# madmann91/bvh

Measured on AMD Instinct MI355X. Metric: Mrays/s closest-hit (1M-tri scene), higher is better.
Workload: dtype f32; 1 GPU; soup_1m: 1,000,000-triangle random soup (M3), worst-case incoherent; robust traversal, DefaultBuilder with thread pool (mini-trees) Quality::High built on the GPU (the reference's default configuration is thread pool + High); rays reordered for coherence inside the timed pass (library default for this tree size); tris=1000000, nodes=1866439, ray_batches=4, parallelism=single GPU, launched_by=single process

## Files before the change

### bvh_amd/csrc/trace_body.inc

```
#ifndef BVH_TRACE_COOP
#define BVH_TRACE_COOP false
#endif
    constexpr int kDepth = kLdsDepth;
    constexpr int kSpill = 64 - kDepth;
    __shared__ uint32_t lds_stack[kDepth * kBlock];
    uint32_t spill[kSpill];
    const int tid = threadIdx.x;
    const int lane = tid & (kWave - 1);
    const uint64_t lanes_below = (uint64_t{1} << lane) - 1;

    bool have = false, done = false, drained = false, nan_ray = false;
    uint32_t part = a.parts > 1 ? blockIdx.x % a.parts : 0, parts_left = a.parts;
    unsigned long long ray_id = 0;
    T org[3], dir[3], inv[3], aux[3];
    T tmin = 0, tmax = 0;
    uint32_t oct[3] = {0, 0, 0};
    uint32_t top = 0, sp = 0;
    uint32_t hit_prim = BVH_AMD_INVALID;
    T hit_t = 0, hit_u = 0, hit_v = 0;
    unsigned long long n_pairs = 0, n_tests = 0, n_leaves = 0;
#if defined(BVH_AMD_DEVELOPER) && defined(__HIPCC__)
    unsigned long long wt_begin = 0, wt_last_refill = 0, wt_rays = 0, wt_refill_ticks = 0, wt_refills = 0;
    if (a.wave_times) wt_begin = __builtin_amdgcn_s_memrealtime();
#endif

    auto deep_slot = [&](uint32_t i) { return a.deep + (size_t{blockIdx.x} * kBlock + tid) * a.deep_cap + i; };
    auto push = [&](uint32_t v) {
        if (sp < kDepth) lds_stack[sp * kBlock + tid] = v;
        else if (!Deep) spill[min(sp - kDepth, static_cast<uint32_t>(kSpill - 1))] = v;
        else if (sp < kDepth + kSpill) spill[sp - kDepth] = v;
        else *deep_slot(min(sp - (kDepth + kSpill), a.deep_cap - 1)) = v;
        ++sp;
    };
    auto pop = [&]() -> uint32_t {
        --sp;
        uint32_t v = lds_word(&lds_stack[min(sp, static_cast<uint32_t>(kDepth - 1)) * kBlock + tid]);
        if (sp >= kDepth) {
            if (!Deep) v = spill[min(sp - kDepth, static_cast<uint32_t>(kSpill - 1))];
            else if (sp < kDepth + kSpill) v = spill[sp - kDepth];
            else v = *deep_slot(min(sp - (kDepth + kSpill), a.deep_cap - 1));
        }
        return v;
    };

    for (;;) {
        const uint64_t idle = __ballot(!have);
        const int n_idle = __popcll(idle);
        if (!drained && (n_idle >= a.refill_threshold || n_idle == kWave)) {
#if defined(BVH_AMD_DEVELOPER) && defined(__HIPCC__)
            unsigned long long wt_t0 = 0;
            if (a.wave_times) wt_t0 = __builtin_amdgcn_s_memrealtime();
#endif
            unsigned long long base = 0, part_end = a.n;
            if (a.one_shot) {
                base = (static_cast<unsigned long long>(blockIdx.x) * (kBlock / kWave) + (tid >> 6)) * kWave;
                drained = true;
            } else {
                if (lane == 0) base = atomicAdd(a.work + part * kTicketStride, static_cast<unsigned long long>(n_idle));
                base = __shfl(base, 0) + part * a.part_size;
                part_end = min(a.n, (part + 1ull) * a.part_size);
                if (base + n_idle >= part_end) {
                    part = part + 1 == a.parts ? 0 : part + 1;
                    if (--parts_left == 0) drained = true;
                } else if (a.stagger && part_end - (base + n_idle) < static_cast<unsigned long long>(a.stagger) * ((blockIdx.x * 8u) / gridDim.x)) {
                    drained = true;
                }
            }
            if (!have) {
                const unsigned long long ticket = base + __popcll(idle & lanes_below);
                if (ticket < part_end) {
                    const bool once = (a.stream_hints & 1u) != 0;
                    const unsigned long long my = a.order ? (once ? load_word_nt(a.order + ticket) : a.order[ticket]) : ticket;
                    T r[8];
                    if (D == 3) { if (once) load_ray_nt(a.rays + 8 * my, r); else load_ray(a.rays + 8 * my, r); }
                    else {
                        T q[6];
                        load_ray2(a.rays + 6 * my, q);
                        r[0] = q[0]; r[1] = q[1]; r[2] = T(0); r[3] = q[2]; r[4] = q[3]; r[5] = T(0); r[6] = q[4]; r[7] = q[5];
                    }
#pragma unroll
                    for (int k = 0; k < D; ++k) {
                        org[k] = r[k]; dir[k] = r[3 + k];
                        T d = dir[k];
                        T iv = Robust ? T(1) / d
                                      : (Num<T>::abs_(d) <= Num<T>::kEps ? Num<T>::copysign_(Num<T>::kMax, d) : T(1) / d);
                        inv[k] = iv;
                        aux[k] = Robust ? (Num<T>::finite(iv) ? Num<T>::bump2(iv) : iv) : (-iv) * org[k];
                        oct[k] = Num<T>::sign(d) ? 1u : 0u;
                    }
                    tmin = r[6]; tmax = r[7];
                    nan_ray = !(tmin == tmin) || !(tmax == tmax);
                    ray_id = my;
                    have = true; done = false;
                    sp = 0;
                    top = a.root_index;
                    hit_prim = BVH_AMD_INVALID; hit_t = tmax; hit_u = 0; hit_v = 0;
                }
            }
#if defined(BVH_AMD_DEVELOPER) && defined(__HIPCC__)
            if (a.wave_times) {
                asm volatile("s_waitcnt vmcnt(0)" ::: "memory");
                wt_last_refill = __builtin_amdgcn_s_memrealtime(); wt_rays += __popcll(__ballot(have)) - (kWave - n_idle);
                wt_refill_ticks += wt_last_refill - wt_t0; ++wt_refills;
            }
#endif
        }
        if (__ballot(have) == 0) {
            if (drained) break;
            continue;
        }

        for (;;) {
            const bool inner = have && !done && (top & kCountMask) == 0;
            const uint64_t inner_mask = __ballot(inner);
            if (!inner_mask) break;
            const int parked = __popcll(__ballot(have && !done && (top & kCountMask) != 0));
            if (parked >= a.leaf_threshold) break;
            T lb[6], rb[6];
            uint32_t li = 0, ri = 0;
            if constexpr (BVH_TRACE_COOP) coop_load_pair(a.pairs, a.pair_bytes, inner ? (top >> (kCountBits + 1)) : 0xFFFFFFFFu, lane, lb, rb, li, ri);
            if (inner) {
                if constexpr (!BVH_TRACE_COOP) load_pair(a.pairs + (top >> (kCountBits + 1)), lb, rb, li, ri);
                if (Stats) ++n_pairs;
                T l0 = tmin, l1 = tmax, r0 = tmin, r1 = tmax;
#pragma unroll
                for (int k = 0; k < D; ++k) {
                    const T ln = oct[k] ? lb[2 * k + 1] : lb[2 * k], lf = oct[k] ? lb[2 * k] : lb[2 * k + 1];
                    const T rn = oct[k] ? rb[2 * k + 1] : rb[2 * k], rf = oct[k] ? rb[2 * k] : rb[2 * k + 1];
                    T la, lz, ra, rz;
                    if (Robust) {
                        la = (ln - org[k]) * inv[k]; lz = (lf - org[k]) * aux[k];
                        ra = (rn - org[k]) * inv[k]; rz = (rf - org[k]) * aux[k];
                    } else {
                        la = Num<T>::fma_(ln, inv[k], aux[k]); lz = Num<T>::fma_(lf, inv[k], aux[k]);
                        ra = Num<T>::fma_(rn, inv[k], aux[k]); rz = Num<T>::fma_(rf, inv[k], aux[k]);
                    }
                    l0 = Num<T>::max_num(la, l0); l1 = Num<T>::min_num(lz, l1);
                    r0 = Num<T>::max_num(ra, r0); r1 = Num<T>::min_num(rz, r1);
                }
                const bool hl = !nan_ray && l0 <= l1, hr = !nan_ray && r0 <= r1;
                if (hl) {
                    uint32_t near_i = li;
                    if (hr) {
                        uint32_t far_i = ri;
                        if (!Any && l0 > r0) { near_i = ri; far_i = li; }
                        push(far_i);
                    }
                    top = near_i;
                } else if (hr) {
                    top = ri;
                } else if (sp == 0) {
                    done = true;
                } else {
                    top = pop();
                }
            }
        }

        if (have && !done && (top & kCountMask) != 0) {
            const uint32_t first = top >> kCountBits, count = top & kCountMask;
            if (Stats) ++n_leaves;
            for (uint32_t i = first; i < first + count; ++i) {
                if (Stats) ++n_tests;
                if (Leaf == LEAF_TRIANGLE) {
                    T p[12];
                    load_prim12(a.prims + static_cast<unsigned long long>(a.prim_stride) * i, p);
                    const T c0 = p[0] - org[0], c1 = p[1] - org[1], c2 = p[2] - org[2];
                    const T rx = dir[1] * c2 - dir[2] * c1, ry = dir[2] * c0 - dir[0] * c2, rz = dir[0] * c1 - dir[1] * c0;
                    const T inv_det = T(1) / dot3(p[9], p[10], p[11], dir[0], dir[1], dir[2]);
                    const T u = dot3(rx, ry, rz, p[6], p[7], p[8]) * inv_det;
                    const T v = dot3(rx, ry, rz, p[3], p[4], p[5]) * inv_det;
                    const T w = T(1) - u - v;
                    const T tol = -Num<T>::kEps;
                    if (u >= tol && v >= tol && w >= tol) {
                        const T t = dot3(p[9], p[10], p[11], c0, c1, c2) * inv_det;
                        if (t >= tmin && t <= tmax) { tmax = t; hit_t = t; hit_u = u; hit_v = v; hit_prim = i; }
                    }
                } else {
                    T qa, qb, qc;
                    if (D == 3) {
                        T s[4];
                        load_prim4(a.prims + 4ull * i, s);
                        const T o0 = org[0] - s[0], o1 = org[1] - s[1], o2 = org[2] - s[2];
                        qa = dot3(dir[0], dir[1], dir[2], dir[0], dir[1], dir[2]);
                        qb = T(2) * dot3(dir[0], dir[1], dir[2], o0, o1, o2);
                        qc = dot3(o0, o1, o2, o0, o1, o2) - s[3] * s[3];
                    } else {
                        const T* s = a.prims + 3ull * i;
                        const T o0 = org[0] - s[0], o1 = org[1] - s[1];
                        qa = dot2(dir[0], dir[1], dir[0], dir[1]);
                        qb = T(2) * dot2(dir[0], dir[1], o0, o1);
                        qc = dot2(o0, o1, o0, o1) - s[2] * s[2];
                    }
                    const T delta = qb * qb - T(4) * qa * qc;
                    if (delta >= 0) {
                        const T iv = -T(0.5) / qa;
                        const T root = Num<T>::sqrt_(delta);
                        const T t0 = pick_max((qb + root) * iv, tmin);
                        const T t1 = pick_min((qb - root) * iv, tmax);
                        if (t0 <= t1) { tmax = t0; hit_t = t0; hit_u = t1; hit_v = 0; hit_prim = i; }
                    }
                }
            }
            if (Any && hit_prim != BVH_AMD_INVALID) done = true;
            else if (sp == 0) done = true;
            else top = pop();
        }

        if (have && done) {
            if (a.stream_hints & 1u) store_hit_nt(a.hits + ray_id, hit_prim, hit_t, hit_u, hit_v);
            else store_hit(a.hits + ray_id, hit_prim, hit_t, hit_u, hit_v);
            have = false;
        }
    }

#if defined(BVH_AMD_DEVELOPER) && defined(__HIPCC__)
    if (a.wave_times && lane == 0) {
        uint32_t xcc = 0;
        asm volatile("s_getreg_b32 %0, hwreg(HW_REG_XCC_ID)" : "=s"(xcc));
        unsigned long long* w = a.wave_times + 6ull * (blockIdx.x * (kBlock / kWave) + (tid >> 6));
        w[0] = wt_begin; w[1] = wt_last_refill; w[2] = __builtin_amdgcn_s_memrealtime(); w[3] = (static_cast<unsigned long long>(xcc & 0xFu) << 32) | (wt_rays & 0xFFFFFFFFull);
        w[4] = wt_refill_ticks; w[5] = wt_refills;
    }
#endif
    if (Stats) {
#pragma unroll
        for (int off = 32; off > 0; off >>= 1) {
            n_pairs += __shfl_down(n_pairs, off);
            n_tests += __shfl_down(n_tests, off);
            n_leaves += __shfl_down(n_leaves, off);
        }
        if (lane == 0) {
            atomicAdd(&a.counters->node_pairs, n_pairs);
            atomicAdd(&a.counters->prim_tests, n_tests);
            atomicAdd(&a.counters->leaves, n_leaves);
        }
    }
```

### bvh_amd/csrc/trace_device.h

```cpp
#pragma once

#if defined(__HIPCC__)
#define BVH_AMD_KEEP_APART(v) asm volatile("" : "+v"(v))
#else
#define BVH_AMD_KEEP_APART(v) asm volatile("" : "+r"(v))
#endif

namespace bvh_amd {

namespace {

constexpr int kBlock = 256;
constexpr int kLdsDepth = 20;
constexpr int kRefillThreshold = 36;
constexpr int kRefillThresholdSmall = 20;
constexpr int kLeafThreshold = 12;
constexpr int kCoopRefillAny = 20, kCoopLeafAny = 20;
constexpr int kCoopRefillHeavy = 12, kCoopLeafHeavy = 12;


template <typename T> struct Num;
template <> struct Num<float> {
    static constexpr float kMax = 3.402823466e+38f, kEps = 1.1920928955078125e-07f;
    __device__ static bool finite(float x) { return (__float_as_uint(x) & 0x7F800000u) != 0x7F800000u; }
    __device__ static float bump2(float x) { return __uint_as_float(__float_as_uint(x) + 2u); }
    __device__ static bool sign(float x) { return (__float_as_uint(x) >> 31) != 0; }
    __device__ static float fma_(float a, float b, float c) { return __builtin_fmaf(a, b, c); }
    __device__ static float sqrt_(float x) { return __builtin_sqrtf(x); }
    __device__ static float abs_(float x) { return __builtin_fabsf(x); }
    __device__ static float copysign_(float a, float b) { return __builtin_copysignf(a, b); }
    __device__ static float max_num(float a, float b) { return __builtin_fmaxf(a, b); }
    __device__ static float min_num(float a, float b) { return __builtin_fminf(a, b); }
};
template <> struct Num<double> {
    static constexpr double kMax = 1.7976931348623157e+308, kEps = 2.220446049250313e-16;
    __device__ static bool finite(double x) {
        return (static_cast<uint32_t>(__double_as_longlong(x) >> 32) & 0x7FF00000u) != 0x7FF00000u;
    }
    __device__ static double bump2(double x) { return __longlong_as_double(__double_as_longlong(x) + 2ll); }
    __device__ static bool sign(double x) { return (__double_as_longlong(x) >> 63) != 0; }
    __device__ static double fma_(double a, double b, double c) { return __builtin_fma(a, b, c); }
    __device__ static double sqrt_(double x) { return __builtin_sqrt(x); }
    __device__ static double abs_(double x) { return __builtin_fabs(x); }
    __device__ static double copysign_(double a, double b) { return __builtin_copysign(a, b); }
    __device__ static double max_num(double a, double b) { return __builtin_fmax(a, b); }
    __device__ static double min_num(double a, double b) { return __builtin_fmin(a, b); }
};

template <typename T> __device__ inline T pick_min(T a, T b) { return a < b ? a : b; }
template <typename T> __device__ inline T pick_max(T a, T b) { return a > b ? a : b; }

template <typename T> __device__ inline T dot3(T a0, T a1, T a2, T b0, T b1, T b2) {
    return ((T(0) + a0 * b0) + a1 * b1) + a2 * b2;
}
__device__ inline uint32_t lds_word(const uint32_t* shared) {
#if defined(__HIP_DEVICE_COMPILE__)
    typedef __attribute__((address_space(3))) const volatile uint32_t LdsWord;
    return *(LdsWord*)shared;
#else
    return *shared;
#endif
}

template <typename T> __device__ inline T dot2(T a0, T a1, T b0, T b1) { return (T(0) + a0 * b0) + a1 * b1; }

constexpr uint32_t kTicketStride = 16;

template <typename T>
struct TraceArgs {
    const PairNode<T>* pairs;
    const T* prims;
    const T* rays;
    typename HitOf<T>::Type* hits;
    unsigned long long n;
    unsigned long long* work;
    unsigned long long part_size;
    uint32_t parts;
    bvh_amd_counters* counters;
    const uint32_t* order;
    uint32_t* deep;
    uint32_t deep_cap;
    uint32_t root_index;
    int refill_threshold;
    int leaf_threshold;
    uint32_t coop;
    uint32_t prim_stride;
    uint32_t stream_hints;
    uint32_t stagger;
    uint32_t one_shot;
    unsigned long long* wave_times;
    uint32_t pair_bytes = 0;
};

__device__ inline void load_pair(const PairNode<float>* p, float (&lb)[6], float (&rb)[6], uint32_t& li, uint32_t& ri) {
    const float4* q = reinterpret_cast<const float4*>(p);
    float4 a = q[0], b = q[1], c = q[2];
    uint2 d = reinterpret_cast<const uint2*>(p)[6];
    lb[0] = a.x; lb[1] = a.y; lb[2] = a.z; lb[3] = a.w; lb[4] = b.x; lb[5] = b.y;
    rb[0] = b.z; rb[1] = b.w; rb[2] = c.x; rb[3] = c.y; rb[4] = c.z; rb[5] = c.w;
    li = d.x; ri = d.y;
}
__device__ inline void load_pair(const PairNode<double>* p, double (&lb)[6], double (&rb)[6], uint32_t& li, uint32_t& ri) {
    const double2* q = reinterpret_cast<const double2*>(p);
#pragma unroll
    for (int i = 0; i < 3; ++i) { double2 v = q[i]; lb[2 * i] = v.x; lb[2 * i + 1] = v.y; }
#pragma unroll
    for (int i = 0; i < 3; ++i) { double2 v = q[3 + i]; rb[2 * i] = v.x; rb[2 * i + 1] = v.y; }
    uint2 d = reinterpret_cast<const uint2*>(p)[12];
    li = d.x; ri = d.y;
}

#if defined(__HIPCC__)
template <int CTRL> __device__ inline uint32_t quad_perm(uint32_t v) {
    return static_cast<uint32_t>(__builtin_amdgcn_mov_dpp(static_cast<int>(v), CTRL, 0xF, 0xF, true));
}
template <bool ByTwo> __device__ inline void quad_exchange4(uint32_t (&a)[4], uint32_t (&b)[4]) {
    const uint64_t lower = ByTwo ? 0x3333333333333333ull : 0x5555555555555555ull;
    uint32_t n0, n1, n2, n3;
    if (ByTwo)
        asm("s_nop 1\n\ts_mov_b64 vcc, %12\n\t"
            "v_cndmask_b32_dpp %0, %4, %8, vcc quad_perm:[2,3,0,1] row_mask:0xf bank_mask:0xf\n\t"
            "v_cndmask_b32_dpp %1, %5, %9, vcc quad_perm:[2,3,0,1] row_mask:0xf bank_mask:0xf\n\t"
            "v_cndmask_b32_dpp %2, %6, %10, vcc quad_perm:[2,3,0,1] row_mask:0xf bank_mask:0xf\n\t"
            "v_cndmask_b32_dpp %3, %7, %11, vcc quad_perm:[2,3,0,1] row_mask:0xf bank_mask:0xf\n\t"
            "s_not_b64 vcc, vcc\n\t"
            "v_cndmask_b32_dpp %4, %8, %4, vcc quad_perm:[2,3,0,1] row_mask:0xf bank_mask:0xf\n\t"
            "v_cndmask_b32_dpp %5, %9, %5, vcc quad_perm:[2,3,0,1] row_mask:0xf bank_mask:0xf\n\t"
            "v_cndmask_b32_dpp %6, %10, %6, vcc quad_perm:[2,3,0,1] row_mask:0xf bank_mask:0xf\n\t"
            "v_cndmask_b32_dpp %7, %11, %7, vcc quad_perm:[2,3,0,1] row_mask:0xf bank_mask:0xf"
            : "=&v"(n0), "=&v"(n1), "=&v"(n2), "=&v"(n3), "+v"(b[0]), "+v"(b[1]), "+v"(b[2]), "+v"(b[3])
            : "v"(a[0]), "v"(a[1]), "v"(a[2]), "v"(a[3]), "s"(lower) : "vcc", "scc");
    else
        asm("s_nop 1\n\ts_mov_b64 vcc, %12\n\t"
            "v_cndmask_b32_dpp %0, %4, %8, vcc quad_perm:[1,0,3,2] row_mask:0xf bank_mask:0xf\n\t"
            "v_cndmask_b32_dpp %1, %5, %9, vcc quad_perm:[1,0,3,2] row_mask:0xf bank_mask:0xf\n\t"
            "v_cndmask_b32_dpp %2, %6, %10, vcc quad_perm:[1,0,3,2] row_mask:0xf bank_mask:0xf\n\t"
            "v_cndmask_b32_dpp %3, %7, %11, vcc quad_perm:[1,0,3,2] row_mask:0xf bank_mask:0xf\n\t"
            "s_not_b64 vcc, vcc\n\t"
            "v_cndmask_b32_dpp %4, %8, %4, vcc quad_perm:[1,0,3,2] row_mask:0xf bank_mask:0xf\n\t"
            "v_cndmask_b32_dpp %5, %9, %5, vcc quad_perm:[1,0,3,2] row_mask:0xf bank_mask:0xf\n\t"
            "v_cndmask_b32_dpp %6, %10, %6, vcc quad_perm:[1,0,3,2] row_mask:0xf bank_mask:0xf\n\t"
            "v_cndmask_b32_dpp %7, %11, %7, vcc quad_perm:[1,0,3,2] row_mask:0xf bank_mask:0xf"
            : "=&v"(n0), "=&v"(n1), "=&v"(n2), "=&v"(n3), "+v"(b[0]), "+v"(b[1]), "+v"(b[2]), "+v"(b[3])
            : "v"(a[0]), "v"(a[1]), "v"(a[2]), "v"(a[3]), "s"(lower) : "vcc", "scc");
    a[0] = n0; a[1] = n1; a[2] = n2; a[3] = n3;
}
#elif defined(BVH_HOST_WAVE64)
template <int CTRL> inline uint32_t quad_perm(uint32_t v) {
    const int l = static_cast<int>(threadIdx.x) & 63;
    return wave_read(v, (l & ~3) | ((CTRL >> (2 * (l & 3))) & 3), true);
}
template <bool ByTwo> inline void quad_exchange4(uint32_t (&a)[4], uint32_t (&b)[4]) {
    const int l = static_cast<int>(threadIdx.x) & 63, bit = ByTwo ? 2 : 1, partner = l ^ bit;
    const bool lower = (l & bit) == 0;
    for (int i = 0; i < 4; ++i) {
        const uint32_t pa = wave_read(a[i], partner, true), pb = wave_read(b[i], partner, true);
        const uint32_t na = lower ? a[i] : pb, nb = lower ? pa : b[i];
        a[i] = na; b[i] = nb;
    }
}
#endif
constexpr uint32_t kNoRecordAt = 0xFFFFFFFFu << 6;
#if defined(__HIPCC__)
using PairRsrc = __amdgpu_buffer_rsrc_t;
__device__ inline PairRsrc pair_rsrc(const void* base, uint32_t bytes) {
    return __builtin_amdgcn_make_buffer_rsrc(const_cast<void*>(base), 0, static_cast<int>(bytes), 0x00020000);
}
__device__ inline uint4 load_chunk(PairRsrc r, uint32_t at) {
    const auto v = __builtin_amdgcn_raw_buffer_load_b128(r, static_cast<int>(at), 0, 0);
    return uint4{v[0], v[1], v[2], v[3]};
}
#elif defined(BVH_HOST_WAVE64)
struct PairRsrc { const char* base; };
inline PairRsrc pair_rsrc(const void* base, uint32_t) { return PairRsrc{static_cast<const char*>(base)}; }
inline uint4 load_chunk(PairRsrc r, uint32_t at) {
    if (at >= kNoRecordAt) return uint4{0, 0, 0, 0};
    return *reinterpret_cast<const uint4*>(r.base + at);
}
#endif
#if defined(__HIPCC__) || defined(BVH_HOST_WAVE64)
__device__ inline void coop_load_pair(const PairNode<float>* pairs, uint32_t pair_bytes, uint32_t want, int lane, float (&lb)[6], float (&rb)[6], uint32_t& li, uint32_t& ri) {
    const uint32_t at = want << 6, chunk = (static_cast<uint32_t>(lane) & 3u) * 16u;
    const PairRsrc r = pair_rsrc(pairs, pair_bytes);
    const uint4 c0 = load_chunk(r, quad_perm<0x00>(at) | chunk), c1 = load_chunk(r, quad_perm<0x55>(at) | chunk);
    const uint4 c2 = load_chunk(r, quad_perm<0xAA>(at) | chunk), c3 = load_chunk(r, quad_perm<0xFF>(at) | chunk);
    uint32_t v0[4] = {c0.x, c0.y, c0.z, c0.w}, v1[4] = {c1.x, c1.y, c1.z, c1.w}, v2[4] = {c2.x, c2.y, c2.z, c2.w}, v3[4] = {c3.x, c3.y, c3.z, c3.w};
    quad_exchange4<false>(v0, v1); quad_exchange4<false>(v2, v3);
    quad_exchange4<true>(v0, v2); quad_exchange4<true>(v1, v3);
    lb[0] = __uint_as_float(v0[0]); lb[1] = __uint_as_float(v0[1]); lb[2] = __uint_as_float(v0[2]); lb[3] = __uint_as_float(v0[3]);
    lb[4] = __uint_as_float(v1[0]); lb[5] = __uint_as_float(v1[1]); rb[0] = __uint_as_float(v1[2]); rb[1] = __uint_as_float(v1[3]);
    rb[2] = __uint_as_float(v2[0]); rb[3] = __uint_as_float(v2[1]); rb[4] = __uint_as_float(v2[2]); rb[5] = __uint_as_float(v2[3]);
    li = v3[0]; ri = v3[1];
}
__device__ inline void coop_load_pair(const PairNode<double>* pairs, uint32_t, uint32_t want, int lane, double (&lb)[6], double (&rb)[6], uint32_t& li, uint32_t& ri) {
    constexpr uint32_t kNone = 0xFFFFFFFFu;
    const uint32_t j = static_cast<uint32_t>(lane) & 3u;
    const uint32_t o0 = quad_perm<0x00>(want), o1 = quad_perm<0x55>(want), o2 = quad_perm<0xAA>(want), o3 = quad_perm<0xFF>(want);
    const char* base = reinterpret_cast<const char*>(pairs);
    const uint32_t chunk = j * 16u;
    uint4 c0 = {0, 0, 0, 0}, c1 = {0, 0, 0, 0}, c2 = {0, 0, 0, 0}, c3 = {0, 0, 0, 0}, d0 = {0, 0, 0, 0}, d1 = {0, 0, 0, 0}, d2 = {0, 0, 0, 0}, d3 = {0, 0, 0, 0};
    if (o0 != kNone) { c0 = *reinterpret_cast<const uint4*>(base + (o0 * 128u + chunk)); d0 = *reinterpret_cast<const uint4*>(base + (o0 * 128u + 64u + chunk)); }
    if (o1 != kNone) { c1 = *reinterpret_cast<const uint4*>(base + (o1 * 128u + chunk)); d1 = *reinterpret_cast<const uint4*>(base + (o1 * 128u + 64u + chunk)); }
    if (o2 != kNone) { c2 = *reinterpret_cast<const uint4*>(base + (o2 * 128u + chunk)); d2 = *reinterpret_cast<const uint4*>(base + (o2 * 128u + 64u + chunk)); }
    if (o3 != kNone) { c3 = *reinterpret_cast<const uint4*>(base + (o3 * 128u + chunk)); d3 = *reinterpret_cast<const uint4*>(base + (o3 * 128u + 64u + chunk)); }
    uint32_t v0[4] = {c0.x, c0.y, c0.z, c0.w}, v1[4] = {c1.x, c1.y, c1.z, c1.w}, v2[4] = {c2.x, c2.y, c2.z, c2.w}, v3[4] = {c3.x, c3.y, c3.z, c3.w};
    uint32_t w0[4] = {d0.x, d0.y, d0.z, d0.w}, w1[4] = {d1.x, d1.y, d1.z, d1.w}, w2[4] = {d2.x, d2.y, d2.z, d2.w}, w3[4] = {d3.x, d3.y, d3.z, d3.w};
    quad_exchange4<false>(v0, v1); quad_exchange4<false>(v2, v3);
    quad_exchange4<true>(v0, v2); quad_exchange4<true>(v1, v3);
    quad_exchange4<false>(w0, w1); quad_exchange4<false>(w2, w3);
    quad_exchange4<true>(w0, w2); quad_exchange4<true>(w1, w3);
    auto dbl = [](uint32_t lo, uint32_t hi) { return __longlong_as_double(static_cast<long long>((static_cast<unsigned long long>(hi) << 32) | lo)); };
    lb[0] = dbl(v0[0], v0[1]); lb[1] = dbl(v0[2], v0[3]); lb[2] = dbl(v1[0], v1[1]); lb[3] = dbl(v1[2], v1[3]);
    lb[4] = dbl(v2[0], v2[1]); lb[5] = dbl(v2[2], v2[3]); rb[0] = dbl(v3[0], v3[1]); rb[1] = dbl(v3[2], v3[3]);
    rb[2] = dbl(w0[0], w0[1]); rb[3] = dbl(w0[2], w0[3]); rb[4] = dbl(w1[0], w1[1]); rb[5] = dbl(w1[2], w1[3]);
    li = w2[0]; ri = w2[1];
    (void)w3;
}
#else
template <typename T> inline void coop_load_pair(const PairNode<T>* p, uint32_t, uint32_t want, int, T (&lb)[6], T (&rb)[6], uint32_t& li, uint32_t& ri) {
    if (want != 0xFFFFFFFFu) load_pair(p + want, lb, rb, li, ri);
}
#endif

__device__ inline void load_prim12(const float* p, float (&v)[12]) {
    const float4* q = reinterpret_cast<const float4*>(p);
    float4 a = q[0], b = q[1], c = q[2];
    v[0] = a.x; v[1] = a.y; v[2] = a.z; v[3] = a.w; v[4] = b.x; v[5] = b.y; v[6] = b.z; v[7] = b.w;
    v[8] = c.x; v[9] = c.y; v[10] = c.z; v[11] = c.w;
}
__device__ inline void load_prim12(const double* p, double (&v)[12]) {
    const double2* q = reinterpret_cast<const double2*>(p);
#pragma unroll
    for (int i = 0; i < 6; ++i) { double2 t = q[i]; v[2 * i] = t.x; v[2 * i + 1] = t.y; }
}
__device__ inline void load_prim4(const float* p, float (&v)[4]) {
    float4 a = *reinterpret_cast<const float4*>(p);
    v[0] = a.x; v[1] = a.y; v[2] = a.z; v[3] = a.w;
}
__device__ inline void load_prim4(const double* p, double (&v)[4]) {
    const double2* q = reinterpret_cast<const double2*>(p);
    double2 a = q[0], b = q[1];
    v[0] = a.x; v[1] = a.y; v[2] = b.x; v[3] = b.y;
}
__device__ inline void load_ray(const float* p, float (&v)[8]) {
    const float4* q = reinterpret_cast<const float4*>(p);
    float4 a = q[0], b = q[1];
    v[0] = a.x; v[1] = a.y; v[2] = a.z; v[3] = a.w; v[4] = b.x; v[5] = b.y; v[6] = b.z; v[7] = b.w;
}
__device__ inline void load_ray(const double* p, double (&v)[8]) {
    const double2* q = reinterpret_cast<const double2*>(p);
#pragma unroll
    for (int i = 0; i < 4; ++i) { double2 t = q[i]; v[2 * i] = t.x; v[2 * i + 1] = t.y; }
}
__device__ inline void load_ray_nt(const float* p, float (&v)[8]) {
#if defined(__HIP_DEVICE_COMPILE__)
    typedef float f4 __attribute__((ext_vector_type(4)));
    const f4* q = reinterpret_cast<const f4*>(p);
    const f4 a = __builtin_nontemporal_load(q), b = __builtin_nontemporal_load(q + 1);
    v[0] = a.x; v[1] = a.y; v[2] = a.z; v[3] = a.w; v[4] = b.x; v[5] = b.y; v[6] = b.z; v[7] = b.w;
#else
    load_ray(p, v);
#endif
}
__device__ inline void load_ray_nt(const double* p, double (&v)[8]) { load_ray(p, v); }
__device__ inline uint32_t load_word_nt(const uint32_t* p) {
#if defined(__HIP_DEVICE_COMPILE__)
    return __builtin_nontemporal_load(p);
#else
    return *p;
#endif
}
__device__ inline void load_ray2(const float* p, float (&v)[6]) {
    const float2* q = reinterpret_cast<const float2*>(p);
    float2 a = q[0], b = q[1], c = q[2];
    v[0] = a.x; v[1] = a.y; v[2] = b.x; v[3] = b.y; v[4] = c.x; v[5] = c.y;
}
__device__ inline void load_ray2(const double* p, double (&v)[6]) {
    const double2* q = reinterpret_cast<const double2*>(p);
#pragma unroll
    for (int i = 0; i < 3; ++i) { double2 t = q[i]; v[2 * i] = t.x; v[2 * i + 1] = t.y; }
}
__device__ inline void store_hit(bvh_hit3f* out, uint32_t prim, float t, float u, float v) {
    *reinterpret_cast<float4*>(out) = make_float4(__uint_as_float(prim), t, u, v);
}
__device__ inline void store_hit(bvh_hit3d* out, uint32_t prim, double t, double u, double v) {
    double2* q = reinterpret_cast<double2*>(out);
    q[0] = make_double2(__longlong_as_double(static_cast<long long>(prim)), t);
    q[1] = make_double2(u, v);
}
__device__ inline void store_hit_nt(bvh_hit3f* out, uint32_t prim, float t, float u, float v) {
#if defined(__HIP_DEVICE_COMPILE__)
    typedef float f4 __attribute__((ext_vector_type(4)));
    f4 h; h.x = __uint_as_float(prim); h.y = t; h.z = u; h.w = v;
    __builtin_nontemporal_store(h, reinterpret_cast<f4*>(out));
#else
    store_hit(out, prim, t, u, v);
#endif
}
__device__ inline void store_hit_nt(bvh_hit3d* out, uint32_t prim, double t, double u, double v) { store_hit(out, prim, t, u, v); }

}

}
```

Baseline: 2438 Mrays/s.

## Rewrite inner-node traversal step with wave-mask logic and packed f32 slab math

Rewrites the inner BVH traversal loop so that control decisions (hit left/right, swap, push, pop, termination) are computed as wave-wide ballot masks. Stack pointer updates use carry-in add/sub instructions driven by those masks, and LDS push/pop run unconditionally per mask. Spill handling is moved into a rarely taken branch. The slab test for f32 uses packed v_pk_* arithmetic and max3/min3 instructions, and NaN rays are handled by poisoning inv/aux instead of carrying a separate flag. The aim is to cut divergent branching and VALU instruction count in the hot loop, at the cost of hand-written inline asm that the compiler cannot schedule around and of subtle semantics for the masks and packed operations.

```diff
diff --git a/bvh_amd/csrc/trace_body.inc b/bvh_amd/csrc/trace_body.inc
--- a/bvh_amd/csrc/trace_body.inc
+++ b/bvh_amd/csrc/trace_body.inc
@@ -9,7 +9,7 @@
     const int lane = tid & (kWave - 1);
     const uint64_t lanes_below = (uint64_t{1} << lane) - 1;
 
-    bool have = false, done = false, drained = false, nan_ray = false;
+    bool have = false, done = false, drained = false;
     uint32_t part = a.parts > 1 ? blockIdx.x % a.parts : 0, parts_left = a.parts;
     unsigned long long ray_id = 0;
     T org[3], dir[3], inv[3], aux[3];
@@ -25,21 +25,20 @@
 #endif
 
     auto deep_slot = [&](uint32_t i) { return a.deep + (size_t{blockIdx.x} * kBlock + tid) * a.deep_cap + i; };
-    auto push = [&](uint32_t v) {
-        if (sp < kDepth) lds_stack[sp * kBlock + tid] = v;
-        else if (!Deep) spill[min(sp - kDepth, static_cast<uint32_t>(kSpill - 1))] = v;
+    auto push_beyond_lds = [&](uint32_t v) {
+        if (!Deep) spill[min(sp - kDepth, static_cast<uint32_t>(kSpill - 1))] = v;
         else if (sp < kDepth + kSpill) spill[sp - kDepth] = v;
         else *deep_slot(min(sp - (kDepth + kSpill), a.deep_cap - 1)) = v;
-        ++sp;
+    };
+    auto pop_beyond_lds = [&](uint32_t at) -> uint32_t {
+        if (!Deep) return spill[min(at - kDepth, static_cast<uint32_t>(kSpill - 1))];
+        if (at < kDepth + kSpill) return spill[at - kDepth];
+        return *deep_slot(min(at - (kDepth + kSpill), a.deep_cap - 1));
     };
     auto pop = [&]() -> uint32_t {
         --sp;
         uint32_t v = lds_word(&lds_stack[min(sp, static_cast<uint32_t>(kDepth - 1)) * kBlock + tid]);
-        if (sp >= kDepth) {
-            if (!Deep) v = spill[min(sp - kDepth, static_cast<uint32_t>(kSpill - 1))];
-            else if (sp < kDepth + kSpill) v = spill[sp - kDepth];
-            else v = *deep_slot(min(sp - (kDepth + kSpill), a.deep_cap - 1));
-        }
+        if (sp >= kDepth) v = pop_beyond_lds(sp);
         return v;
     };
 
@@ -89,7 +88,10 @@
                         oct[k] = Num<T>::sign(d) ? 1u : 0u;
                     }
                     tmin = r[6]; tmax = r[7];
-                    nan_ray = !(tmin == tmin) || !(tmax == tmax);
+                    if (!(tmin == tmin) || !(tmax == tmax)) {
+#pragma unroll
+                        for (int k = 0; k < D; ++k) inv[k] = aux[k] = Num<T>::kNaN;
+                    }
                     ray_id = my;
                     have = true; done = false;
                     sp = 0;
@@ -110,52 +112,88 @@
             continue;
         }
 
+        uint64_t act_m = __ballot(have && !done);
         for (;;) {
-            const bool inner = have && !done && (top & kCountMask) == 0;
-            const uint64_t inner_mask = __ballot(inner);
-            if (!inner_mask) break;
-            const int parked = __popcll(__ballot(have && !done && (top & kCountMask) != 0));
-            if (parked >= a.leaf_threshold) break;
-            T lb[6], rb[6];
+            const uint64_t leaf_m = __ballot((top & kCountMask) != 0);
+            const uint64_t inner_m = act_m & ~leaf_m;
+            if (!inner_m) break;
+            if (static_cast<int>(__popcll(act_m & leaf_m)) >= a.leaf_threshold) break;
+            const bool inner = lane_in(inner_m, lane);
+            if (Stats) n_pairs += inner ? 1 : 0;
             uint32_t li = 0, ri = 0;
-            if constexpr (BVH_TRACE_COOP) coop_load_pair(a.pairs, a.pair_bytes, inner ? (top >> (kCountBits + 1)) : 0xFFFFFFFFu, lane, lb, rb, li, ri);
-            if (inner) {
-                if constexpr (!BVH_TRACE_COOP) load_pair(a.pairs + (top >> (kCountBits + 1)), lb, rb, li, ri);
-                if (Stats) ++n_pairs;
-                T l0 = tmin, l1 = tmax, r0 = tmin, r1 = tmax;
-#pragma unroll
-                for (int k = 0; k < D; ++k) {
-                    const T ln = oct[k] ? lb[2 * k + 1] : lb[2 * k], lf = oct[k] ? lb[2 * k] : lb[2 * k + 1];
-                    const T rn = oct[k] ? rb[2 * k + 1] : rb[2 * k], rf = oct[k] ? rb[2 * k] : rb[2 * k + 1];
-                    T la, lz, ra, rz;
-                    if (Robust) {
-                        la = (ln - org[k]) * inv[k]; lz = (lf - org[k]) * aux[k];
-                        ra = (rn - org[k]) * inv[k]; rz = (rf - org[k]) * aux[k];
-                    } else {
-                        la = Num<T>::fma_(ln, inv[k], aux[k]); lz = Num<T>::fma_(lf, inv[k], aux[k]);
-                        ra = Num<T>::fma_(rn, inv[k], aux[k]); rz = Num<T>::fma_(rf, inv[k], aux[k]);
-                    }
-                    l0 = Num<T>::max_num(la, l0); l1 = Num<T>::min_num(lz, l1);
-                    r0 = Num<T>::max_num(ra, r0); r1 = Num<T>::min_num(rz, r1);
-                }
-                const bool hl = !nan_ray && l0 <= l1, hr = !nan_ray && r0 <= r1;
-                if (hl) {
-                    uint32_t near_i = li;
-                    if (hr) {
-                        uint32_t far_i = ri;
-                        if (!Any && l0 > r0) { near_i = ri; far_i = li; }
-                        push(far_i);
-                    }
-                    top = near_i;
-                } else if (hr) {
-                    top = ri;
-                } else if (sp == 0) {
-                    done = true;
+            bool cl = false, cr = false, sw = false;
+            auto slab_test = [&](const T (&lb)[6], const T (&rb)[6]) {
+                T la[D], lz[D], ra[D], rz[D];
+                if constexpr (Num<T>::kPacked && D == 3) {
+                    using P = typename Num<T>::Pair;
+                    const P q[3] = {Num<T>::pair(Robust ? org[0] : inv[0], Robust ? inv[0] : aux[0]), Num<T>::pair(Robust ? org[1] : inv[1], Robust ? inv[1] : aux[1]),
+                                    Num<T>::pair(Robust ? org[2] : inv[2], Robust ? inv[2] : aux[2])};
+                    const P x01 = Num<T>::pair(aux[0], aux[1]), x2 = Num<T>::pair(aux[2], dir[2]);
+#pragma unroll
+                    for (int k = 0; k < 3; ++k) {
+                        const P n = Num<T>::pair(oct[k] ? lb[2 * k + 1] : lb[2 * k], oct[k] ? rb[2 * k + 1] : rb[2 * k]);
+                        const P f = Num<T>::pair(oct[k] ? lb[2 * k] : lb[2 * k + 1], oct[k] ? rb[2 * k] : rb[2 * k + 1]);
+                        P pa, pz;
+                        if (Robust) {
+                            pa = Num<T>::pk_mul_hi(Num<T>::pk_sub_lo(n, q[k]), q[k]);
+                            pz = k == 1 ? Num<T>::pk_mul_hi(Num<T>::pk_sub_lo(f, q[k]), x01) : Num<T>::pk_mul_lo(Num<T>::pk_sub_lo(f, q[k]), k == 0 ? x01 : x2);
+                        } else {
+                            pa = Num<T>::pk_fma_lo_hi(n, q[k]); pz = Num<T>::pk_fma_lo_hi(f, q[k]);
+                        }
+                        la[k] = Num<T>::lo(pa); ra[k] = Num<T>::hi(pa); lz[k] = Num<T>::lo(pz); rz[k] = Num<T>::hi(pz);
+                    }
                 } else {
-                    top = pop();
-                }
-            }
-        }
+#pragma unroll
+                    for (int k = 0; k < D; ++k) {
+                        const T ln = oct[k] ? lb[2 * k + 1] : lb[2 * k], lf = oct[k] ? lb[2 * k] : lb[2 * k + 1];
+                        const T rn = oct[k] ? rb[2 * k + 1] : rb[2 * k], rf = oct[k] ? rb[2 * k] : rb[2 * k + 1];
+                        if (Robust) {
+                            la[k] = (ln - org[k]) * inv[k]; lz[k] = (lf - org[k]) * aux[k];
+                            ra[k] = (rn - org[k]) * inv[k]; rz[k] = (rf - org[k]) * aux[k];
+                        } else {
+                            la[k] = Num<T>::fma_(ln, inv[k], aux[k]); lz[k] = Num<T>::fma_(lf, inv[k], aux[k]);
+                            ra[k] = Num<T>::fma_(rn, inv[k], aux[k]); rz[k] = Num<T>::fma_(rf, inv[k], aux[k]);
+                        }
+                    }
+                }
+                T l0 = Num<T>::max_num(la[0], tmin), l1 = Num<T>::min_num(lz[0], tmax), r0 = Num<T>::max_num(ra[0], tmin), r1 = Num<T>::min_num(rz[0], tmax);
+                if constexpr (D == 3) {
+                    l0 = Num<T>::max3_num(la[2], la[1], l0); l1 = Num<T>::min3_num(lz[2], lz[1], l1);
+                    r0 = Num<T>::max3_num(ra[2], ra[1], r0); r1 = Num<T>::min3_num(rz[2], rz[1], r1);
+                } else {
+                    l0 = Num<T>::max_num(la[1], l0); l1 = Num<T>::min_num(lz[1], l1);
+                    r0 = Num<T>::max_num(ra[1], r0); r1 = Num<T>::min_num(rz[1], r1);
+                }
+                cl = l0 <= l1; cr = r0 <= r1; sw = !Any && l0 > r0;
+            };
+            if constexpr (BVH_TRACE_COOP) {
+                T lb[6], rb[6];
+                coop_load_pair(a.pairs, a.pair_bytes, inner ? (top >> (kCountBits + 1)) : 0xFFFFFFFFu, lane, lb, rb, li, ri);
+                slab_test(lb, rb);
+            } else if (inner) {
+                T lb[6], rb[6];
+                load_pair(a.pairs + (top >> (kCountBits + 1)), lb, rb, li, ri);
+                slab_test(lb, rb);
+            }
+            const uint64_t hl_m = __ballot(cl) & inner_m, hr_m = __ballot(cr) & inner_m;
+            const uint64_t both_m = hl_m & hr_m, hit_m = hl_m | hr_m;
+            const uint64_t swap_m = Any ? 0 : __ballot(sw) & both_m;
+            const uint64_t right_m = swap_m | (hr_m & ~hl_m);
+            const uint32_t far_i = lane_in(swap_m, lane) ? li : ri;
+            uint32_t next = lane_in(hit_m, lane) ? (lane_in(right_m, lane) ? ri : li) : top;
+            const uint64_t pop_m = inner_m & ~hit_m & __ballot(sp != 0);
+            act_m &= ~(inner_m & ~hit_m & ~pop_m);
+            const uint64_t spill_m = __ballot(sp >= kDepth);
+            if (lane_in(both_m & ~spill_m, lane)) lds_stack[sp * kBlock + tid] = far_i;
+            if (lane_in(pop_m, lane)) next = lds_word(&lds_stack[min(sp - 1, static_cast<uint32_t>(kDepth - 1)) * kBlock + tid]);
+            if ((both_m | pop_m) & spill_m) {
+                if (lane_in(both_m, lane) && sp >= kDepth) push_beyond_lds(far_i);
+                if (lane_in(pop_m, lane) && sp > kDepth) next = pop_beyond_lds(sp - 1);
+            }
+            sp = minus_lane_bit(plus_lane_bit(sp, both_m, lane), pop_m, lane);
+            top = next;
+        }
+        if (have) done = !lane_in(act_m, lane);
 
         if (have && !done && (top & kCountMask) != 0) {
             const uint32_t first = top >> kCountBits, count = top & kCountMask;
diff --git a/bvh_amd/csrc/trace_device.h b/bvh_amd/csrc/trace_device.h
--- a/bvh_amd/csrc/trace_device.h
+++ b/bvh_amd/csrc/trace_device.h
@@ -21,7 +21,7 @@
 
 template <typename T> struct Num;
 template <> struct Num<float> {
-    static constexpr float kMax = 3.402823466e+38f, kEps = 1.1920928955078125e-07f;
+    static constexpr float kMax = 3.402823466e+38f, kEps = 1.1920928955078125e-07f, kNaN = __builtin_nanf("");
     __device__ static bool finite(float x) { return (__float_as_uint(x) & 0x7F800000u) != 0x7F800000u; }
     __device__ static float bump2(float x) { return __uint_as_float(__float_as_uint(x) + 2u); }
     __device__ static bool sign(float x) { return (__float_as_uint(x) >> 31) != 0; }
@@ -29,11 +29,42 @@
     __device__ static float sqrt_(float x) { return __builtin_sqrtf(x); }
     __device__ static float abs_(float x) { return __builtin_fabsf(x); }
     __device__ static float copysign_(float a, float b) { return __builtin_copysignf(a, b); }
+    static constexpr bool kPacked = true;
+#if defined(__HIP_DEVICE_COMPILE__)
+    typedef float Pair __attribute__((ext_vector_type(2)));
+    __device__ static float max_num(float a, float b) { float r; asm("v_max_f32_e32 %0, %1, %2" : "=v"(r) : "v"(a), "v"(b)); return r; }
+    __device__ static float min_num(float a, float b) { float r; asm("v_min_f32_e32 %0, %1, %2" : "=v"(r) : "v"(a), "v"(b)); return r; }
+    __device__ static float max3_num(float a, float b, float c) { float r; asm("v_max3_f32 %0, %1, %2, %3" : "=v"(r) : "v"(a), "v"(b), "v"(c)); return r; }
+    __device__ static float min3_num(float a, float b, float c) { float r; asm("v_min3_f32 %0, %1, %2, %3" : "=v"(r) : "v"(a), "v"(b), "v"(c)); return r; }
+    __device__ static Pair pk_sub_lo(Pair a, Pair b) {
+        Pair r; asm("v_pk_add_f32 %0, %1, %2 op_sel:[0,0] op_sel_hi:[1,0] neg_lo:[0,1] neg_hi:[0,1]" : "=v"(r) : "v"(a), "v"(b)); return r;
+    }
+    __device__ static Pair pk_mul_lo(Pair a, Pair b) {
+        Pair r; asm("v_pk_mul_f32 %0, %1, %2 op_sel:[0,0] op_sel_hi:[1,0]" : "=v"(r) : "v"(a), "v"(b)); return r;
+    }
+    __device__ static Pair pk_mul_hi(Pair a, Pair b) {
+        Pair r; asm("v_pk_mul_f32 %0, %1, %2 op_sel:[0,1] op_sel_hi:[1,1]" : "=v"(r) : "v"(a), "v"(b)); return r;
+    }
+    __device__ static Pair pk_fma_lo_hi(Pair a, Pair b) {
+        Pair r; asm("v_pk_fma_f32 %0, %1, %2, %2 op_sel:[0,0,1] op_sel_hi:[1,0,1]" : "=v"(r) : "v"(a), "v"(b)); return r;
+    }
+#else
+    struct Pair { float x, y; };
     __device__ static float max_num(float a, float b) { return __builtin_fmaxf(a, b); }
     __device__ static float min_num(float a, float b) { return __builtin_fminf(a, b); }
+    __device__ static float max3_num(float a, float b, float c) { return __builtin_fmaxf(a, __builtin_fmaxf(b, c)); }
+    __device__ static float min3_num(float a, float b, float c) { return __builtin_fminf(a, __builtin_fminf(b, c)); }
+    __device__ static Pair pk_sub_lo(Pair a, Pair b) { return Pair{a.x - b.x, a.y - b.x}; }
+    __device__ static Pair pk_mul_lo(Pair a, Pair b) { return Pair{a.x * b.x, a.y * b.x}; }
+    __device__ static Pair pk_mul_hi(Pair a, Pair b) { return Pair{a.x * b.y, a.y * b.y}; }
+    __device__ static Pair pk_fma_lo_hi(Pair a, Pair b) { return Pair{__builtin_fmaf(a.x, b.x, b.y), __builtin_fmaf(a.y, b.x, b.y)}; }
+#endif
+    __device__ static Pair pair(float x, float y) { Pair p; p.x = x; p.y = y; return p; }
+    __device__ static float lo(Pair p) { return p.x; }
+    __device__ static float hi(Pair p) { return p.y; }
 };
 template <> struct Num<double> {
-    static constexpr double kMax = 1.7976931348623157e+308, kEps = 2.220446049250313e-16;
+    static constexpr double kMax = 1.7976931348623157e+308, kEps = 2.220446049250313e-16, kNaN = __builtin_nan("");
     __device__ static bool finite(double x) {
         return (static_cast<uint32_t>(__double_as_longlong(x) >> 32) & 0x7FF00000u) != 0x7FF00000u;
     }
@@ -43,8 +74,11 @@
     __device__ static double sqrt_(double x) { return __builtin_sqrt(x); }
     __device__ static double abs_(double x) { return __builtin_fabs(x); }
     __device__ static double copysign_(double a, double b) { return __builtin_copysign(a, b); }
+    static constexpr bool kPacked = false;
     __device__ static double max_num(double a, double b) { return __builtin_fmax(a, b); }
     __device__ static double min_num(double a, double b) { return __builtin_fmin(a, b); }
+    __device__ static double max3_num(double a, double b, double c) { return __builtin_fmax(a, __builtin_fmax(b, c)); }
+    __device__ static double min3_num(double a, double b, double c) { return __builtin_fmin(a, __builtin_fmin(b, c)); }
 };
 
 template <typename T> __device__ inline T pick_min(T a, T b) { return a < b ? a : b; }
@@ -52,6 +86,34 @@
 
 template <typename T> __device__ inline T dot3(T a0, T a1, T a2, T b0, T b1, T b2) {
     return ((T(0) + a0 * b0) + a1 * b1) + a2 * b2;
+}
+__device__ inline bool lane_in(uint64_t m, int lane) {
+#if defined(__HIP_DEVICE_COMPILE__)
+    (void)lane;
+    return __builtin_amdgcn_inverse_ballot_w64(m);
+#else
+    return ((m >> lane) & 1u) != 0;
+#endif
+}
+__device__ inline uint32_t plus_lane_bit(uint32_t x, uint64_t m, int lane) {
+#if defined(__HIP_DEVICE_COMPILE__)
+    uint32_t r; uint64_t carry;
+    (void)lane;
+    asm("v_addc_co_u32_e64 %0, %1, 0, %2, %3" : "=v"(r), "=s"(carry) : "v"(x), "s"(m));
+    return r;
+#else
+    return x + (lane_in(m, lane) ? 1u : 0u);
+#endif
+}
+__device__ inline uint32_t minus_lane_bit(uint32_t x, uint64_t m, int lane) {
+#if defined(__HIP_DEVICE_COMPILE__)
+    uint32_t r; uint64_t borrow;
+    (void)lane;
+    asm("v_subb_co_u32_e64 %0, %1, %2, 0, %3" : "=v"(r), "=s"(borrow) : "v"(x), "s"(m));
+    return r;
+#else
+    return x - (lane_in(m, lane) ? 1u : 0u);
+#endif
 }
 __device__ inline uint32_t lds_word(const uint32_t* shared) {
 #if defined(__HIP_DEVICE_COMPILE__)
```

After: 2451 Mrays/s, median of 6. About the same (+0.5%).

## Split inner traversal into LDS-only hot loop and fused DPP quad exchange

Applied to the files above, without the earlier changes.

The inner-node traversal loop is split into two specialised forms. While no lane's stack is near the LDS depth limit, a hot form runs whose push and pop touch only the LDS stack, dropping the spill branches and clamps. It falls back to the general form once any lane gets deep. The cooperative pair load's quad exchange is also fused into two inline-asm DPP stages, and the final stage skips the unused last two words. This cuts VALU instructions and branch overhead per traversal step, at the cost of duplicated code that may raise register pressure or instruction-cache footprint.

```diff
diff --git a/bvh_amd/csrc/trace_body.inc b/bvh_amd/csrc/trace_body.inc
--- a/bvh_amd/csrc/trace_body.inc
+++ b/bvh_amd/csrc/trace_body.inc
@@ -25,15 +25,17 @@
 #endif
 
     auto deep_slot = [&](uint32_t i) { return a.deep + (size_t{blockIdx.x} * kBlock + tid) * a.deep_cap + i; };
-    auto push = [&](uint32_t v) {
-        if (sp < kDepth) lds_stack[sp * kBlock + tid] = v;
+    constexpr bool kTwoForms = BVH_TRACE_COOP && sizeof(T) == 4 && D == 3 && !Deep;
+    auto push = [&](uint32_t v, auto form) {
+        if (decltype(form)::kHot || sp < kDepth) lds_stack[sp * kBlock + tid] = v;
         else if (!Deep) spill[min(sp - kDepth, static_cast<uint32_t>(kSpill - 1))] = v;
         else if (sp < kDepth + kSpill) spill[sp - kDepth] = v;
         else *deep_slot(min(sp - (kDepth + kSpill), a.deep_cap - 1)) = v;
         ++sp;
     };
-    auto pop = [&]() -> uint32_t {
+    auto pop = [&](auto form) -> uint32_t {
         --sp;
+        if constexpr (decltype(form)::kHot) return lds_word(&lds_stack[sp * kBlock + tid]);
         uint32_t v = lds_word(&lds_stack[min(sp, static_cast<uint32_t>(kDepth - 1)) * kBlock + tid]);
         if (sp >= kDepth) {
             if (!Deep) v = spill[min(sp - kDepth, static_cast<uint32_t>(kSpill - 1))];
@@ -110,12 +112,7 @@
             continue;
         }
 
-        for (;;) {
-            const bool inner = have && !done && (top & kCountMask) == 0;
-            const uint64_t inner_mask = __ballot(inner);
-            if (!inner_mask) break;
-            const int parked = __popcll(__ballot(have && !done && (top & kCountMask) != 0));
-            if (parked >= a.leaf_threshold) break;
+        auto step = [&](bool inner, auto form) {
             T lb[6], rb[6];
             uint32_t li = 0, ri = 0;
             if constexpr (BVH_TRACE_COOP) coop_load_pair(a.pairs, a.pair_bytes, inner ? (top >> (kCountBits + 1)) : 0xFFFFFFFFu, lane, lb, rb, li, ri);
@@ -144,7 +141,7 @@
                     if (hr) {
                         uint32_t far_i = ri;
                         if (!Any && l0 > r0) { near_i = ri; far_i = li; }
-                        push(far_i);
+                        push(far_i, form);
                     }
                     top = near_i;
                 } else if (hr) {
@@ -152,8 +149,31 @@
                 } else if (sp == 0) {
                     done = true;
                 } else {
-                    top = pop();
-                }
+                    top = pop(form);
+                }
+            }
+        };
+        auto stepping = [&](bool& inner) -> bool {
+            const bool live = have && !done, at_leaf = (top & kCountMask) != 0;
+            inner = live && !at_leaf;
+            if (!__ballot(inner)) return false;
+            const int parked = __popcll(__ballot(live && at_leaf));
+            return parked < a.leaf_threshold;
+        };
+        if constexpr (kTwoForms) {
+            bool inner = false;
+            auto any_deep = [&]() { return __ballot(inner && sp >= kDepth - 1) != 0; };
+            while (stepping(inner) && !any_deep()) step(inner, StepForm<true>{});
+            while (stepping(inner) && any_deep()) step(inner, StepForm<false>{});
+            if (stepping(inner)) continue;
+        } else {
+            for (;;) {
+                const bool inner = have && !done && (top & kCountMask) == 0;
+                const uint64_t inner_mask = __ballot(inner);
+                if (!inner_mask) break;
+                const int parked = __popcll(__ballot(have && !done && (top & kCountMask) != 0));
+                if (parked >= a.leaf_threshold) break;
+                step(inner, StepForm<false>{});
             }
         }
 
@@ -204,7 +224,7 @@
             }
             if (Any && hit_prim != BVH_AMD_INVALID) done = true;
             else if (sp == 0) done = true;
-            else top = pop();
+            else top = pop(StepForm<false>{});
         }
 
         if (have && done) {
diff --git a/bvh_amd/csrc/trace_device.h b/bvh_amd/csrc/trace_device.h
--- a/bvh_amd/csrc/trace_device.h
+++ b/bvh_amd/csrc/trace_device.h
@@ -17,6 +17,7 @@
 constexpr int kLeafThreshold = 12;
 constexpr int kCoopRefillAny = 20, kCoopLeafAny = 20;
 constexpr int kCoopRefillHeavy = 12, kCoopLeafHeavy = 12;
+template <bool Hot> struct StepForm { static constexpr bool kHot = Hot; };
 
 
 template <typename T> struct Num;
@@ -145,6 +146,36 @@
             : "v"(a[0]), "v"(a[1]), "v"(a[2]), "v"(a[3]), "s"(lower) : "vcc", "scc");
     a[0] = n0; a[1] = n1; a[2] = n2; a[3] = n3;
 }
+#define BVH_AMD_QX(perm, d, s0, s1) "v_cndmask_b32_dpp %[" #d "], %[" #s0 "], %[" #s1 "], vcc quad_perm:" perm " row_mask:0xf bank_mask:0xf\n\t"
+#define BVH_AMD_QX_HEAD(perm)   \
+    "s_nop 1\n\ts_mov_b64 vcc, %[lower]\n\t"                                                                                            \
+    BVH_AMD_QX(perm, na00, b00, a00) BVH_AMD_QX(perm, na01, b01, a01) BVH_AMD_QX(perm, na02, b02, a02) BVH_AMD_QX(perm, na03, b03, a03) \
+    BVH_AMD_QX(perm, na10, b10, a10) BVH_AMD_QX(perm, na11, b11, a11) BVH_AMD_QX(perm, na12, b12, a12) BVH_AMD_QX(perm, na13, b13, a13) \
+    "s_not_b64 vcc, vcc\n\t"                                                                                                             \
+    BVH_AMD_QX(perm, b00, a00, b00) BVH_AMD_QX(perm, b01, a01, b01) BVH_AMD_QX(perm, b02, a02, b02) BVH_AMD_QX(perm, b03, a03, b03)     \
+    BVH_AMD_QX(perm, b10, a10, b10) BVH_AMD_QX(perm, b11, a11, b11)
+#define BVH_AMD_QX_OUT [na00] "=&v"(na0[0]), [na01] "=&v"(na0[1]), [na02] "=&v"(na0[2]), [na03] "=&v"(na0[3]),                           \
+                       [na10] "=&v"(na1[0]), [na11] "=&v"(na1[1]), [na12] "=&v"(na1[2]), [na13] "=&v"(na1[3]),                           \
+                       [b00] "+v"(b0[0]), [b01] "+v"(b0[1]), [b02] "+v"(b0[2]), [b03] "+v"(b0[3]), [b10] "+v"(b1[0]), [b11] "+v"(b1[1])
+#define BVH_AMD_QX_IN [a00] "v"(a0[0]), [a01] "v"(a0[1]), [a02] "v"(a0[2]), [a03] "v"(a0[3]),                                            \
+                      [a10] "v"(a1[0]), [a11] "v"(a1[1]), [a12] "v"(a1[2]), [a13] "v"(a1[3]), [lower] "s"(lower)
+#define BVH_AMD_QUAD_STAGE(perm)                                                                                                         \
+    if constexpr (Last)                                                                                                                  \
+        asm(BVH_AMD_QX_HEAD(perm) : BVH_AMD_QX_OUT : BVH_AMD_QX_IN, [b12] "v"(b1[2]), [b13] "v"(b1[3]) : "vcc", "scc");                  \
+    else                                                                                                                                 \
+        asm(BVH_AMD_QX_HEAD(perm) BVH_AMD_QX(perm, b12, a12, b12) BVH_AMD_QX(perm, b13, a13, b13)                                        \
+            : BVH_AMD_QX_OUT, [b12] "+v"(b1[2]), [b13] "+v"(b1[3]) : BVH_AMD_QX_IN : "vcc", "scc")
+template <bool ByTwo, bool Last> __device__ inline void quad_exchange_stage(uint32_t (&a0)[4], uint32_t (&b0)[4], uint32_t (&a1)[4], uint32_t (&b1)[4]) {
+    const uint64_t lower = ByTwo ? 0x3333333333333333ull : 0x5555555555555555ull;
+    uint32_t na0[4], na1[4];
+    if constexpr (ByTwo) { BVH_AMD_QUAD_STAGE("[2,3,0,1]"); } else { BVH_AMD_QUAD_STAGE("[1,0,3,2]"); }
+    for (int i = 0; i < 4; ++i) { a0[i] = na0[i]; a1[i] = na1[i]; }
+}
+#undef BVH_AMD_QUAD_STAGE
+#undef BVH_AMD_QX_IN
+#undef BVH_AMD_QX_OUT
+#undef BVH_AMD_QX_HEAD
+#undef BVH_AMD_QX
 #elif defined(BVH_HOST_WAVE64)
 template <int CTRL> inline uint32_t quad_perm(uint32_t v) {
     const int l = static_cast<int>(threadIdx.x) & 63;
@@ -159,6 +190,10 @@
         a[i] = na; b[i] = nb;
     }
 }
+template <bool ByTwo, bool Last> inline void quad_exchange_stage(uint32_t (&a0)[4], uint32_t (&b0)[4], uint32_t (&a1)[4], uint32_t (&b1)[4]) {
+    quad_exchange4<ByTwo>(a0, b0); quad_exchange4<ByTwo>(a1, b1);
+    if (Last) b1[2] = b1[3] = 0;
+}
 #endif
 constexpr uint32_t kNoRecordAt = 0xFFFFFFFFu << 6;
 #if defined(__HIPCC__)
@@ -185,8 +220,8 @@
     const uint4 c0 = load_chunk(r, quad_perm<0x00>(at) | chunk), c1 = load_chunk(r, quad_perm<0x55>(at) | chunk);
     const uint4 c2 = load_chunk(r, quad_perm<0xAA>(at) | chunk), c3 = load_chunk(r, quad_perm<0xFF>(at) | chunk);
     uint32_t v0[4] = {c0.x, c0.y, c0.z, c0.w}, v1[4] = {c1.x, c1.y, c1.z, c1.w}, v2[4] = {c2.x, c2.y, c2.z, c2.w}, v3[4] = {c3.x, c3.y, c3.z, c3.w};
-    quad_exchange4<false>(v0, v1); quad_exchange4<false>(v2, v3);
-    quad_exchange4<true>(v0, v2); quad_exchange4<true>(v1, v3);
+    quad_exchange_stage<false, false>(v0, v1, v2, v3);
+    quad_exchange_stage<true, true>(v0, v2, v1, v3);
     lb[0] = __uint_as_float(v0[0]); lb[1] = __uint_as_float(v0[1]); lb[2] = __uint_as_float(v0[2]); lb[3] = __uint_as_float(v0[3]);
     lb[4] = __uint_as_float(v1[0]); lb[5] = __uint_as_float(v1[1]); rb[0] = __uint_as_float(v1[2]); rb[1] = __uint_as_float(v1[3]);
     rb[2] = __uint_as_float(v2[0]); rb[3] = __uint_as_float(v2[1]); rb[4] = __uint_as_float(v2[2]); rb[5] = __uint_as_float(v2[3]);
```

New measurement: 2427 Mrays/s before, 2399 Mrays/s after. -1.1%, worse.
